# AugmentariumLab/VolumeRenderer

Hardware: AMD Instinct MI355X
Metric: Mvoxels/s kd-tree compress+decode (higher is better)
Workload: dtype u8; 1 GPU; 2048x2048x1920 uint8 volume per GPU as 960 bricks of 256x256x128, rm_volume, tolerance 1, maxEpochs 2, VolumeKdtree build + levelCut

## Files before the change

volumerenderer_amd/csrc/brickset.h:

```cpp
#pragma once
#include "kd_common.h"
#include "../../include/vrhip.h"
#include <algorithm>
#include <string>
#include <vector>

namespace vr {

struct Stream2 {
    uint8_t *temp = nullptr;
    uint8_t *codes = nullptr;
    uint8_t *recon[3] = {nullptr, nullptr, nullptr};
    Ctrl *ctrl = nullptr;
    uint8_t *tree = nullptr;
    uint8_t *treeCompact = nullptr;
};

struct Switches {
    bool decodeWalk = false;
    bool decodeFineV1 = false;
    bool decodeQuad = false;
    bool noSkipBlocks = false;
    bool noUniformBlocks = false;
    bool noUniformDecode = false;
};

#define VR_LOD_SLOTS 4
struct LodSlot {
    int32_t *dev = nullptr;
    int32_t *host = nullptr;
    uint8_t *idxValCut = nullptr;
    uint32_t *decTables = nullptr;
    uint8_t *rankVals = nullptr;
    int64_t *obDev = nullptr;
    int64_t *obHost = nullptr;
    vr_pool_entry *tabHost = nullptr;
    int64_t tabCap = 0;
    hipEvent_t done = nullptr;
    bool pending = false;
};

struct BrickSet {
    int32_t B = 0;
    Switches sw;
    Geom g{};
    TilePlan tile{};
// ... 108 lines not shown
```

volumerenderer_amd/csrc/capi.hip:

```cpp
#include "../../include/vrhip.h"
#include "brickset.h"
#include "raymarch.h"
#include <math.h>
#include <stdio.h>
#include <stdlib.h>
#include <string.h>
#include <algorithm>
#include <array>
#include <atomic>
#include <map>
#include <mutex>
#include <new>

using namespace vr;

struct vr_brickset { BrickSet s; };

#define HIPCHK(x) do { hipError_t e_ = (x); if (e_ != hipSuccess) return e_ == hipErrorOutOfMemory ? VR_ERR_OOM : VR_ERR_NO_DEVICE; } while (0)

static bool device_ok()
{
    int n = 0;
    hipError_t e = hipGetDeviceCount(&n);
    if ((e != hipSuccess || n <= 0) && getenv("VRHIP_DEBUG"))
// ... 186 lines not shown
static bool misaligned16(const void *p) { return ((uintptr_t)p & 15) != 0; }

vr_status vr_brickset_create(vr_brickset **out, int32_t num_bricks, const int64_t dims[3], int32_t tolerance,
                             int32_t max_epochs, int32_t variant)
{
    if (!out || !dims || num_bricks <= 0) return VR_ERR_INVALID;
    if (tolerance < 0 || max_epochs < 0 || variant < 0 || variant > 2) return VR_ERR_INVALID;
    for (int k = 0; k < 3; ++k) if (dims[k] <= 0) return VR_ERR_INVALID;
    bool general = !pow2(dims[0]) || !pow2(dims[1]) || !pow2(dims[2]) || dims[0] > 1024 || dims[1] > 1024 || dims[2] > 1024;
    if (dims[0] > (1ll << 20) || dims[1] > (1ll << 20) || dims[2] > (1ll << 20) || dims[0] * dims[1] * dims[2] >= (1ll << 32))
        return VR_ERR_UNSUPPORTED;
    if (!device_ok()) return VR_ERR_NO_DEVICE;
    vr_brickset *h = new (std::nothrow) vr_brickset();
    if (!h) return VR_ERR_OOM;
    BrickSet &b = h->s;
    b.B = num_bricks;
    {
        Switches &w = b.sw;
        w.decodeWalk = getenv("VRHIP_DECODE_WALK") != nullptr;
        w.decodeFineV1 = getenv("VRHIP_DECODE_FINE_V1") != nullptr;
        w.decodeQuad = getenv("VRHIP_DECODE_QUAD") != nullptr;
        w.noSkipBlocks = getenv("VRHIP_NO_SKIP_BLOCKS") != nullptr;
        w.noUniformBlocks = getenv("VRHIP_NO_UNIFORM_BLOCKS") != nullptr;
        w.noUniformDecode = getenv("VRHIP_NO_UNIFORM_DECODE") != nullptr;
    }
    make_geom(b.g, dims);
    b.D = b.g.D;
    if (b.D > 31) { delete h; return VR_ERR_UNSUPPORTED; }
    b.idx64 = b.D > 28 || (getenv("VRHIP_FORCE_IDX64") && b.D >= 12);
    if (b.idx64) general = true;
    if (b.idx64 && num_bricks != 1 && b.D > 28) { delete h; return VR_ERR_UNSUPPORTED; }
    b.generalGeom = general;
    b.maxDepth = b.D + VR_CHAIN_LEVELS;
    b.tolerance = tolerance; b.maxEpochs = max_epochs; b.variant = variant;
    b.K = b.D < 6 ? b.D : 6;
    b.Ds = b.D - b.K;
    b.heapStride = (int64_t)1 << (b.D + 1);
    b.leafStride = (int64_t)1 << b.D;
    b.codeStride = ((b.heapStride + 15) / 16) * 4;
    b.reconStride = b.leafStride;
    const int64_t numMax = b.heapStride - 1 + VR_CHAIN_LEVELS * b.leafStride;
    b.treeCap = ((numMax + 15) / 16 + 2) * 4 + 256;
    if (b.D >= 12) {
        const int64_t gappedBytes = ((int64_t)1 << (b.D - 12)) * 2320 * 4 + 256;
        if (gappedBytes > b.treeCap) b.treeCap = gappedBytes;
    }
// ... 15 lines not shown
        if (e == hipSuccess && !general) e = upload(b.lut, make_lut(b.g, b.K));
        if (e == hipSuccess && !general) e = hipMalloc(&b.spread, (size_t)(b.g.X + b.g.Y + b.g.Z) * sizeof(uint32_t));
        if (e == hipSuccess && !general) e = upload(b.spread, make_spread(b.g));
        for (int i = 0; i < 8 && e == hipSuccess; ++i) e = hipEventCreate(&b.ev[i]);
        if (e != hipSuccess) rc = e == hipErrorOutOfMemory ? VR_ERR_OOM : VR_ERR_NO_DEVICE;
    }
    if (rc != VR_OK) { vr_brickset_destroy(h); return rc; }
    b.hostCtrl.resize(b.B);
    b.openTreeBytes.assign(b.B, -1);
    *out = h;
    return VR_OK;
}

vr_status vr_brickset_set_switch(vr_brickset *h, const char *name, int32_t value)
{
    if (!h || !name) return VR_ERR_INVALID;
    Switches &w = h->s.sw;
    const bool on = value != 0;
    if (!strcmp(name, "decode_walk")) w.decodeWalk = on;
    else if (!strcmp(name, "decode_fine_v1")) w.decodeFineV1 = on;
    else if (!strcmp(name, "decode_quad")) w.decodeQuad = on;
    else if (!strcmp(name, "no_skip_blocks")) w.noSkipBlocks = on;
    else if (!strcmp(name, "no_uniform_blocks")) w.noUniformBlocks = on;
    else if (!strcmp(name, "no_uniform_decode")) w.noUniformDecode = on;
    else return VR_ERR_INVALID;
    return VR_OK;
}

vr_status vr_brickset_set_compaction(vr_brickset *h, int32_t on_build)
{
    if (!h) return VR_ERR_INVALID;
    h->s.compactOnBuild = on_build != 0;
    return VR_OK;
}

vr_status vr_debug_set(const char *name, int32_t value)
{
    if (!name) return VR_ERR_INVALID;
    if (!strcmp(name, "skip_grid_v1")) { vr::g_skipGridV1.store(value ? 1 : 0); return VR_OK; }
    if (!strcmp(name, "reslice_tile_w")) {
        if (value != 8 && value != 16 && value != 64) return VR_ERR_INVALID;
        vr::g_resliceTileLog2.store(value == 8 ? 3 : (value == 16 ? 4 : 6));
        return VR_OK;
    }
    if (!strcmp(name, "hist_plain")) { vr::g_histPlain.store(value ? 1 : 0); return VR_OK; }
    return VR_ERR_INVALID;
// ... 1019 lines not shown
```

volumerenderer_amd/csrc/kd_encode.hip:

```cpp
#include "brickset.h"
#include <math.h>
#include <stdio.h>
#include <stdlib.h>
#include <string.h>

namespace vr {

#define FILL_NODES_PER_BLOCK 1024
#define EMIT_RANKS_PER_BLOCK 256

template <bool FROM_VOXELS>
__global__ void __launch_bounds__(256)
k_pyramid(Geom g, int dLeaf, int L, const uint8_t *__restrict__ vox, const uint8_t *__restrict__ inMin,
          const uint8_t *__restrict__ inMax, int64_t inStride, uint8_t *__restrict__ temp, int64_t heapStride,
          uint8_t *__restrict__ tempRange, uint8_t *__restrict__ outMin, uint8_t *__restrict__ outMax,
          int64_t outStride, const uint32_t *__restrict__ srcIdx)
{
    __shared__ uint8_t smn[2][1024], smx[2][1024];
    const int brick = blockIdx.y;
    const uint32_t n = 1u << L;
    const uint32_t base = blockIdx.x << L;
    uint8_t *T = temp + (int64_t)brick * heapStride;
    uint8_t *TR = tempRange ? tempRange + (int64_t)brick * heapStride : nullptr;
    for (uint32_t i = threadIdx.x; i < n; i += blockDim.x) {
// ... 225 lines not shown
            const uint32_t u = pk_u(__builtin_elementwise_min(pk_s(waveMM[2 * h]), pk_s(waveMM[2 * h + 1])));
            a[h] = (int)(u & 0xFFFFu); b[h] = 255 - (int)(u >> 16);
            const int64_t o = ((int64_t)1 << (D - 11)) + (base >> 11) + h;
            T[o] = (uint8_t)((a[h] + b[h]) >> 1);
            if (TR) TR[o] = (uint8_t)((b[h] - a[h]) >> 1);
        }
        const int ra = min(a[0], a[1]), rbm = max(b[0], b[1]);
        const int64_t o = ((int64_t)1 << (D - 12)) + (base >> 12);
        T[o] = (uint8_t)((ra + rbm) >> 1);
        if (TR) TR[o] = (uint8_t)((rbm - ra) >> 1);
        outMin[(int64_t)brick * outStride + (base >> 12)] = (uint8_t)ra;
        outMax[(int64_t)brick * outStride + (base >> 12)] = (uint8_t)rbm;
        if (blockFlag) blockFlag[(int64_t)brick * ((int64_t)1 << (D - 12)) + (base >> 12)] = ra == rbm ? 1u : 0u;
        if (blockFlagR) blockFlagR[(int64_t)brick * ((int64_t)1 << (D - 12)) + (base >> 12)] = ra == rbm ? 1u : 0u;
    }
}

struct ReconBufs { uint8_t *b[3]; };

struct SkipBlocks {
    uint8_t *flag;
    int64_t nBlk;
    int Dm2;
};
__device__ __forceinline__ bool skip_block(const SkipBlocks &sk, int brick, int d, uint32_t node)
{
    return sk.flag && d > sk.Dm2 && (sk.flag[(int64_t)brick * sk.nBlk + (node >> (10 + d - sk.Dm2))] & 2u) != 0u;
}

__device__ inline int phys_buf(const Ctrl &c, int role) { return role == 0 ? c.ra : c.rb; }

__global__ void k_ctrl_init(Ctrl *ctrls, const uint8_t *rootMin, const uint8_t *rootMax, int64_t mmStride)
{
    Ctrl &c = ctrls[blockIdx.x];
    if (threadIdx.x) return;
    c.constBrick = 0; c.constVal = 0; c.zeroRun = 0;
    if (rootMin) {
        const int mn = rootMin[(int64_t)blockIdx.x * mmStride], mx = rootMax[(int64_t)blockIdx.x * mmStride];
        c.constBrick = mn == mx ? 1 : 0;
        c.constVal = mn;
    }
    c.currentDistance = c.currentError = c.currentDF = c.currentStepSize = 0.0;
    c.previousDistance = c.previousError = c.previousDF = c.previousStepSize = 0.0;
    c.errMinus = c.errPlus = 0;
    c.statL1 = 0;
    c.numActive = 0;
    c.epoch = 0; c.active = 0; c.fillThisEpoch = 0;
    c.cur = 0; c.prev = 1; c.pendingEqual = 0;
    c.par = 0; c.ra = 1; c.rb = 2;
    c.altValid = 0; c.altSel = 0; c.altDist = 0;
// ... 10 lines not shown
#define est_at(ci, seg) (((int64_t)(ci) * summStride + (int64_t)(seg)) * 4)

__device__ __forceinline__ uint32_t wave_incl_scan_u32(uint32_t v, int lane)
{
    (void)lane;
    return wave_incl_scan_add_dpp(v);
}

__device__ __forceinline__ uint32_t lane_u32(uint32_t v, int l) { return (uint32_t)__builtin_amdgcn_readlane((int)v, l); }
__device__ __forceinline__ unsigned long long lane_u64(unsigned long long v, int l)
{
    return (unsigned long long)lane_u32((uint32_t)v, l) | ((unsigned long long)lane_u32((uint32_t)(v >> 32), l) << 32);
}

#define EST_STAGE_NODES 4096
__device__ inline void est_exact_chain(const uint8_t *__restrict__ T, const uint8_t *__restrict__ P, int d, uint32_t lo,
                                       uint32_t hi, unsigned long long &S, uint32_t &C, int lane, const SkipBlocks &sk, int brick,
                                       uint8_t *stage = nullptr)
{
    const uint32_t len = hi - lo;
    const bool staged = stage && d > 0 && len >= 64u && len <= (uint32_t)EST_STAGE_NODES && (len & 63u) == 0u && (lo & 31u) == 0u;
    const uint8_t *sT = stage, *sP = stage + EST_STAGE_NODES;
    if (staged) {
        for (uint32_t i = (uint32_t)lane * 16u; i < len; i += 1024u) *(uint4 *)(stage + i) = *(const uint4 *)(T + lo + i);
        for (uint32_t i = (uint32_t)lane * 16u; i < len / 2u; i += 1024u) *(uint4 *)(stage + EST_STAGE_NODES + i) = *(const uint4 *)(P + (lo >> 1) + i);
    }
    const bool sk0 = skip_block(sk, brick, d, lo);
    int tn = 0, pn = 0;
    if (staged) { tn = sT[lane]; pn = sP[lane >> 1]; }
    else { tn = (!sk0 && lo + lane < hi) ? T[lo + lane] : 0; pn = (!sk0 && lo + lane < hi && d > 0) ? P[(lo + lane) >> 1] : 0; }
    bool skipThis = sk0;
    for (uint32_t base = lo; base < hi; base += 64) {
        uint32_t i = base + lane;
        bool valid = i < hi;
        const int t = tn, p = pn;
        const bool skipped = skipThis;
        {
            const uint32_t i2 = i + 64;
            skipThis = base + 64 < hi && skip_block(sk, brick, d, base + 64);
            if (staged) {
                const uint32_t j2 = i2 - lo;
                tn = j2 < len ? sT[j2] : 0;
                pn = j2 < len ? sP[j2 >> 1] : 0;
            } else {
                tn = (!skipThis && i2 < hi) ? T[i2] : 0;
                pn = (!skipThis && i2 < hi && d > 0) ? P[i2 >> 1] : 0;
            }
        }
        if (skipped) continue;
        int pd = p > t ? p - t : t - p;
        bool forced = (t > p && 2 * t - p > 255) || (t < p && 2 * t < p);
        bool cand = valid && pd > 0;
        bool dec = cand && (forced || S < (unsigned long long)pd * (2ull * C + 1ull));
        unsigned long long mask = __ballot(dec);
        for (int it = 0; it < 65; ++it) {
            uint32_t cpre = __popcll(mask & ((1ull << lane) - 1ull));
            uint32_t v = dec ? (uint32_t)pd : 0u;
            uint32_t spre = wave_incl_scan_u32(v, lane) - v;
            bool nd = cand && (forced || (S + spre) < (unsigned long long)pd * (2ull * (C + cpre) + 1ull));
            unsigned long long nmask = __ballot(nd);
            dec = nd;
            if (nmask == mask) break;
            mask = nmask;
        }
        S += (uint32_t)__builtin_amdgcn_readlane((int)wave_incl_scan_add_dpp(dec ? (uint32_t)pd : 0u), 63);
        C += __popcll(mask);
    }
}

// ... 49 lines not shown
    return v + dpp_u32<0x142, 0xa>(0, v);
}
__device__ __forceinline__ int seg_max_i32_dpp(int v)
{
    v = row_max_i32_dpp(v);
    return max(v, (int)dpp_u32<0x142, 0xa>(0x80000000u, (uint32_t)v));
}
__device__ __forceinline__ int seg_min_i32_dpp(int v)
{
    v = row_min_i32_dpp(v);
    return min(v, (int)dpp_u32<0x142, 0xa>(0x7FFFFFFFu, (uint32_t)v));
}

__global__ void __launch_bounds__(256)
k_est_summ(int d, int nc, Ctrl *ctrls, const uint8_t *__restrict__ temp, int64_t heapStride, ReconBufs rb,
           int64_t leafStride, uint32_t *__restrict__ summ, int64_t summStride, SkipBlocks sk)
{
    constexpr int L = 32, SPW = 64 / L, NP = EST_SEG / 2 / L, TW = NP / 2, PW = NP / 4;
    const int brick = blockIdx.y, lane = threadIdx.x & 63, row = lane / L, rl = lane % L;
    const Ctrl &c = ctrls[brick];
    const uint32_t n = 1u << d;
    const int cConst = c.constBrick, cDone = c.estDone, cSeg = c.estSeg, cPar = c.par, cTbase = c.estTbase;
    if (cConst || cDone) return;
    const uint8_t *Tl = temp + (int64_t)brick * heapStride + ((int64_t)1 << d) + rl * (4 * TW);
    const uint8_t *Pl = (cPar == 0 ? rb.b[0] : (cPar == 1 ? rb.b[1] : rb.b[2])) + (int64_t)brick * leafStride + rl * (4 * PW);
    const uint32_t nseg = n / EST_SEG, step = gridDim.x * (4u * SPW);
    const uint32_t g0 = (uint32_t)cSeg + (blockIdx.x * 4u + (threadIdx.x >> 6)) * SPW;
    uint4 tN[TW / 4], pN[PW / 4];
    auto fetch = [&](uint32_t g) {
        const uint32_t s = g + (uint32_t)row;
        const bool live = s < nseg && !skip_block(sk, brick, d, s * EST_SEG);
#pragma unroll
        for (int j = 0; j < TW / 4; ++j) tN[j] = make_uint4(0, 0, 0, 0);
#pragma unroll
        for (int j = 0; j < PW / 4; ++j) pN[j] = make_uint4(0, 0, 0, 0);
        if (live) {
#pragma unroll
            for (int j = 0; j < TW / 4; ++j) tN[j] = ld16(Tl + (size_t)s * EST_SEG + 16 * j);
#pragma unroll
            for (int j = 0; j < PW / 4; ++j) pN[j] = ld16(Pl + (size_t)s * (EST_SEG / 2) + 16 * j);
        }
    };
    fetch(g0);
    const int Tbase = cTbase;
    uint32_t *out = summ + (int64_t)brick * summStride * (4 * EST_CAND);
    for (uint32_t g = g0; g < nseg; g += step) {
    uint32_t tw[TW], pw[PW];
#pragma unroll
    for (int j = 0; j < TW / 4; ++j) { tw[4 * j] = tN[j].x; tw[4 * j + 1] = tN[j].y; tw[4 * j + 2] = tN[j].z; tw[4 * j + 3] = tN[j].w; }
#pragma unroll
    for (int j = 0; j < PW / 4; ++j) { pw[4 * j] = pN[j].x; pw[4 * j + 1] = pN[j].y; pw[4 * j + 2] = pN[j].z; pw[4 * j + 3] = pN[j].w; }
    const uint32_t seg = g + (uint32_t)row;
    const bool segLive = seg < nseg;
    uint32_t mixed = 0;
    {
        const uint32_t t0 = __builtin_amdgcn_perm(0, tw[0], 0u), p0 = __builtin_amdgcn_perm(0, pw[0], 0u);
#pragma unroll
        for (int j = 0; j < TW; ++j) mixed |= tw[j] ^ t0;
#pragma unroll
// ... 255 lines not shown
{
    __shared__ unsigned long long shm[4], shp[4];
    const int brick = blockIdx.y;
    Ctrl &c = ctrls[brick];
    const int cConst = c.constBrick, cFill = c.fillThisEpoch, cPar = c.par, cCur = c.cur, cRa = c.ra, cRb = c.rb, cEpoch = c.epoch;
    const double cDist = c.currentDistance;
    if (cConst || !cFill) return;
    if (!STORE && c.altSel) return;
    const uint8_t *T = temp + (int64_t)brick * heapStride + ((int64_t)1 << d);
    uint8_t *Cd = codes + (int64_t)brick * codeStride + ((int64_t)1 << (d - 2));
    const int rPhys = cCur == 0 ? cRa : cRb;
    const uint8_t *P = (cPar == 0 ? rb.b[0] : (cPar == 1 ? rb.b[1] : rb.b[2])) + (int64_t)brick * leafStride;
    uint8_t *R = (rPhys == 0 ? rb.b[0] : (rPhys == 1 ? rb.b[1] : rb.b[2])) + (int64_t)brick * leafStride;
    const int dist = (int)(uint8_t)cDist;
    const int distM = (int)(uint8_t)fmax(0.0, cDist - 1.0);
    const int distP = (int)(uint8_t)fmin(255.0, cDist + 1.0);
    const bool needDF = cEpoch + 1 < maxEpochs;
    const uint32_t d2 = (uint32_t)dist * 0x10001u, dm2 = (uint32_t)distM * 0x10001u, dp2 = (uint32_t)distP * 0x10001u;
    const int w = threadIdx.x >> 6;
    const uint32_t nchunk = (uint32_t)(((size_t)1 << d) >> 12);
    uint32_t chunk = blockIdx.x * (uint32_t)iters;
    const uint32_t chunkEnd = chunk + (uint32_t)iters < nchunk ? chunk + (uint32_t)iters : nchunk;
    unsigned long long accM = 0, accP = 0;
    bool skippedN = skip_block(sk, brick, d, (chunk * 4u + (uint32_t)w) << 10);
    uint4 tvN = make_uint4(0, 0, 0, 0);
    uint2 pvN = make_uint2(0, 0);
    if (!skippedN) { const size_t i0 = ((size_t)chunk * 256u + threadIdx.x) * 16u; tvN = ld16(T + i0); pvN = ld8(P + (i0 >> 1)); }
    for (; chunk < chunkEnd; ++chunk) {
    const size_t i0 = ((size_t)chunk * 256u + threadIdx.x) * 16u;
    const bool skipped = skippedN;
    const uint4 tv = tvN;
    const uint2 pv = pvN;
    if (chunk + 1 < chunkEnd) {
        skippedN = skip_block(sk, brick, d, ((chunk + 1u) * 4u + (uint32_t)w) << 10);
        tvN = make_uint4(0, 0, 0, 0); pvN = make_uint2(0, 0);
        if (!skippedN) { const size_t i1 = i0 + 4096u; tvN = ld16(T + i1); pvN = ld8(P + (i1 >> 1)); }
    }
    const uint32_t tw[4] = {tv.x, tv.y, tv.z, tv.w}, pw[2] = {pv.x, pv.y};
    uint32_t e0 = 0, em = 0, ep = 0, wa = 0, wb = 0, rw[4] = {tw[0], tw[1], tw[2], tw[3]}, rprev = 0;
    const uint32_t differs = (tw[0] ^ __builtin_amdgcn_perm(0, pw[0], 0x01010000u)) | (tw[1] ^ __builtin_amdgcn_perm(0, pw[0], 0x03030202u)) |
                             (tw[2] ^ __builtin_amdgcn_perm(0, pw[1], 0x01010000u)) | (tw[3] ^ __builtin_amdgcn_perm(0, pw[1], 0x03030202u));
    const bool busy = !skipped && __ballot(differs != 0u) != 0ull;
    if (sk.flag && d == sk.Dm2 && !busy && (threadIdx.x & 63) == 0) {
        uint8_t *f = sk.flag + (int64_t)brick * sk.nBlk + (size_t)chunk * 4 + w;
        if (*f & 1u) *f = 3u;
    }
    const auto pair = [&](const int j) {
        const EncPair c = enc_pair(tw[j >> 1], j & 1, pw[j >> 2], j & 3);
        const vr_s16x2 x = enc_pair_x(c, d2), ax = pk_abs(x);
        e0 = pk_sumsq(__builtin_elementwise_min(c.pd, ax), e0);
        if (STORE) {
        const uint32_t take = pk_u((ax - c.pd) >> 15);
        const uint32_t code2 = take & pk_u(pk_s(c.up) + pk_s(0x00020002u));
        if (j < 4) wa |= code2 << (4 * j); else wb |= code2 << (4 * (j - 4));
        const vr_s16x2 r = pk_mad(x, pk_mad(pk_s(c.up), pk_s(0xFFFEFFFEu), pk_s(0xFFFFFFFFu)), c.T2);
        const uint32_t rec = (take & pk_u(r)) | (~take & pk_u(c.P2));
        if (j & 1) rw[j >> 1] = __builtin_amdgcn_perm(rec, rprev, 0x06040200u); else rprev = rec;
        }
        if (needDF) {
            em = pk_sumsq(enc_pair_err(c, dm2), em);
            ep = pk_sumsq(enc_pair_err(c, dp2), ep);
        }
    };
    bool uniform = false;
    if (busy) {
        const uint32_t t0 = __builtin_amdgcn_perm(0, tw[0], 0u), p0 = __builtin_amdgcn_perm(0, pw[0], 0u);
        const uint32_t mixed = (tw[0] ^ t0) | (tw[1] ^ t0) | (tw[2] ^ t0) | (tw[3] ^ t0) | (pw[0] ^ p0) | (pw[1] ^ p0);
        uniform = __ballot(mixed != 0u) == 0ull;
    }
    if (uniform) {
        pair(0);
        e0 *= 8u; em *= 8u; ep *= 8u;
        if (STORE) {
            wa *= 0x1111u; wb = wa;
            rw[0] = rw[1] = rw[2] = rw[3] = __builtin_amdgcn_perm(0, rprev, 0u);
        }
    } else if (busy)
#pragma unroll
        for (int j = 0; j < 8; ++j) pair(j);
    const uint32_t cpk = ((wa | (wa >> 14)) & 0xFFFFu) | ((wb | (wb >> 14)) << 16);
    if (!skipped && STORE) {
        st4(Cd + (i0 >> 2), cpk);
        st16(R + i0, make_uint4(rw[0], rw[1], rw[2], rw[3]));
    }
    unsigned long long s0 = 0, sm = 0, sp = 0;
    if (busy) {
        s0 = (uint32_t)__builtin_amdgcn_readlane((int)wave_incl_scan_add_dpp(e0), 63);
        sm = (uint32_t)__builtin_amdgcn_readlane((int)wave_incl_scan_add_dpp(em), 63);
        sp = (uint32_t)__builtin_amdgcn_readlane((int)wave_incl_scan_add_dpp(ep), 63);
    }
    if ((threadIdx.x & 63) == 0) {
        blockErr[(int64_t)brick * nErrBlk + (size_t)chunk * 4 + w] = s0;
        if (!STORE && needDF) {
            blockErr[errPlane + (int64_t)brick * nErrBlk + (size_t)chunk * 4 + w] = sm;
            blockErr[2 * errPlane + (int64_t)brick * nErrBlk + (size_t)chunk * 4 + w] = sp;
        }
    }
    accM += sm; accP += sp;
    }
    if ((threadIdx.x & 63) == 0) { shm[w] = accM; shp[w] = accP; }
    __syncthreads();
    if (threadIdx.x == 0) {
        const unsigned long long tm = shm[0] + shm[1] + shm[2] + shm[3], tp = shp[0] + shp[1] + shp[2] + shp[3];
        if (tm) atomicAdd(&c.errMinus, tm);
// ... 25 lines not shown
            int er = encode_node(t, p, dist).err;
            e = (uint32_t)(er * er);
        }
        const uint32_t incl = wave_incl_scan_u32(e, lane);
        const uint32_t total = lane_u32(incl, 63);
        uint32_t consumed = 0;
        int start = 0;
        while (true) {
            bool ok = true;
            if (lane >= start && s != 0.0) ok = (s + (double)(incl - consumed)) < next_pow2_above(s);
            const unsigned long long bad = ~__ballot(ok);
            if (bad == 0ull) { s = s + (double)(total - consumed); break; }
            const int f = __ffsll((long long)bad) - 1;
            const uint32_t exclF = lane_u32(incl - e, f), eF = lane_u32(e, f);
            s = s + (double)(exclF - consumed);
            s = s + (double)eF;
            consumed = exclF + eF;
            start = f + 1;
        }
    }
    return s;
}

__device__ inline double ctl_walk_block16(double s, const uint8_t *__restrict__ T, const uint8_t *__restrict__ P, int dist,
                                          uint32_t lo, int lane)
{
    const uint4 tv = *(const uint4 *)(T + lo + lane * 16);
    const uint2 pv = *(const uint2 *)(P + (lo >> 1) + lane * 8);
    const uint32_t tw[4] = {tv.x, tv.y, tv.z, tv.w}, pw[2] = {pv.x, pv.y};
    const uint32_t d2 = (uint32_t)dist * 0x10001u;
    uint32_t e[16], pre[16];
    uint32_t run = 0;
#pragma unroll
    for (int j = 0; j < 8; ++j) {
        const EncPair c = enc_pair(tw[j >> 1], j & 1, pw[j >> 2], j & 3);
        const vr_s16x2 er = enc_pair_err(c, d2);
        e[2 * j] = (uint32_t)((int)er.x * (int)er.x);
        e[2 * j + 1] = (uint32_t)((int)er.y * (int)er.y);
        run += e[2 * j]; pre[2 * j] = run;
        run += e[2 * j + 1]; pre[2 * j + 1] = run;
    }
    const uint32_t inclL = wave_incl_scan_add_dpp(run);
    const uint32_t baseL = inclL - run, total = (uint32_t)__builtin_amdgcn_readlane((int)inclL, 63);
    uint32_t consumed = 0;
    int startPos = 0;
    while (true) {
        int fail = 16;
        if (s != 0.0) {
            const double bound = next_pow2_above(s);
#pragma unroll
            for (int k = 15; k >= 0; --k)
                if (lane * 16 + k >= startPos && !((s + (double)(baseL + pre[k] - consumed)) < bound)) fail = k;
        }
        const unsigned long long bad = __ballot(fail < 16);
        if (bad == 0ull) { s = s + (double)(total - consumed); break; }
        const int f = __ffsll((long long)bad) - 1;
        const int kF = __builtin_amdgcn_readlane(fail, f);
        uint32_t eF = 0, gF = 0;
#pragma unroll
        for (int k = 0; k < 16; ++k) if (k == kF) { eF = e[k]; gF = baseL + pre[k]; }
        eF = (uint32_t)__builtin_amdgcn_readlane((int)eF, f);
        gF = (uint32_t)__builtin_amdgcn_readlane((int)gF, f);
        s = s + (double)(gF - eF - consumed);
        s = s + (double)eF;
        consumed = gF;
        startPos = f * 16 + kF + 1;
    }
    return s;
}

#define CTL_STAGE_BLOCKS 8192
__device__ inline double ctl_partials64(double s, const unsigned long long *__restrict__ be, const uint32_t *stg, uint32_t base, uint32_t nblk,
                                        const uint8_t *__restrict__ T, const uint8_t *__restrict__ P, int d, int dist,
                                        uint32_t n, int lane)
{
    const unsigned long long e2 = base + lane < nblk ? (stg ? (unsigned long long)stg[base + lane] : be[base + lane]) : 0ull;
    const unsigned long long incl = (unsigned long long)wave_incl_scan_add_dpp((uint32_t)(e2 & 0xFFFFFFull)) +
                                    ((unsigned long long)wave_incl_scan_add_dpp((uint32_t)(e2 >> 24)) << 24);
    const unsigned long long total = lane_u64(incl, 63);
    unsigned long long consumed = 0;
    int start = 0;
    while (true) {
        bool ok = true;
        const bool sInt = (s == floor(s)) && (s + (double)(total - consumed)) < 9007199254740992.0;
        if (lane >= start && !sInt) ok = (s + (double)(incl - consumed)) < next_pow2_above(s);
        const unsigned long long bad = ~__ballot(ok);
        if (bad == 0ull) { s = s + (double)(total - consumed); break; }
        const int f = __ffsll((long long)bad) - 1;
        const unsigned long long exclF = lane_u64(incl - e2, f), inclF = lane_u64(incl, f);
        s = s + (double)(exclF - consumed);
        uint32_t lo = (base + f) * FILL_NODES_PER_BLOCK, hi = lo + FILL_NODES_PER_BLOCK;
        if (hi > n) hi = n;
        s = (hi - lo == 1024u && d > 0) ? ctl_walk_block16(s, T, P, dist, lo, lane) : ctl_walk_block(s, T, P, d, dist, lo, hi, lane);
        consumed = inclF;
        start = f + 1;
    }
    return s;
}

__global__ void __launch_bounds__(64)
k_control(int d, int maxEpochs, int guarded, Ctrl *ctrls, const uint8_t *__restrict__ temp, int64_t heapStride,
          ReconBufs rb, int64_t leafStride, const unsigned long long *__restrict__ blockErr, int64_t nErrBlk, int64_t errPlane,
          int leaflessLeaf)
{
    const int brick = blockIdx.x, lane = threadIdx.x;
    __shared__ __attribute__((aligned(16))) uint32_t ctlStage[CTL_STAGE_BLOCKS];
    Ctrl &c = ctrls[brick];
    if (c.constBrick) return;
    const uint32_t n = 1u << d;
    const bool ending = c.active && c.fillThisEpoch;
    double s = c.currentError;
    if (ending) {
        const uint8_t *T = temp + (int64_t)brick * heapStride + ((int64_t)1 << d);
        const uint8_t *P = rb.b[c.par] + (int64_t)brick * leafStride;
        const int dist = (int)(uint8_t)c.currentDistance;
        const uint32_t nblk = (n + FILL_NODES_PER_BLOCK - 1) / FILL_NODES_PER_BLOCK;
        const unsigned long long *be = blockErr + (int64_t)c.altSel * errPlane + (int64_t)brick * nErrBlk;
        const uint32_t nchunk = (nblk + 63u) >> 6;
        const uint32_t *stg = nullptr;
        if (nblk >= 256u && nblk <= (uint32_t)CTL_STAGE_BLOCKS && (nblk & 255u) == 0u) {
            for (uint32_t i = (uint32_t)lane * 4u; i < nblk; i += 256u) {
                const uint4 a = *(const uint4 *)(be + i), b = *(const uint4 *)(be + i + 2);
                *(uint4 *)(ctlStage + i) = make_uint4(a.x, a.z, b.x, b.z);
            }
            stg = ctlStage;
        }
// ... 7 lines not shown
            } else if (ch < nchunk) {
                const unsigned long long *q = be + (size_t)ch * 64;
                const uint32_t m = nblk - ch * 64 < 64u ? nblk - ch * 64 : 64u;
                if (m == 64u) {
#pragma unroll 8
                    for (int k = 0; k < 64; ++k) tot += q[k];
                } else
                    for (uint32_t k = 0; k < m; ++k) tot += q[k];
            }
            const unsigned long long incl = (unsigned long long)wave_incl_scan_add_dpp((uint32_t)(tot & 0xFFFFFFull)) +
                                            ((unsigned long long)wave_incl_scan_add_dpp((uint32_t)(tot >> 24)) << 24);
            const unsigned long long total = lane_u64(incl, 63);
            unsigned long long consumed = 0;
            int start = 0;
            while (true) {
                bool ok = true;
                const bool sInt = (s == floor(s)) && (s + (double)(total - consumed)) < 9007199254740992.0;
                if (lane >= start && !sInt) ok = (s + (double)(incl - consumed)) < next_pow2_above(s);
                const unsigned long long bad = ~__ballot(ok);
                if (bad == 0ull) { s = s + (double)(total - consumed); break; }
                const int f = __ffsll((long long)bad) - 1;
                const unsigned long long exclF = lane_u64(incl - tot, f), inclF = lane_u64(incl, f);
                s = s + (double)(exclF - consumed);
                s = ctl_partials64(s, be, stg, (cb + (uint32_t)f) * 64u, nblk, T, P, d, dist, n, lane);
                consumed = inclF;
                start = f + 1;
            }
        }
    }
    if (lane != 0) return;
    if (ending) {
        c.roleDist[c.cur] = (int)(uint8_t)c.currentDistance;
        c.codesDist = (int)(uint8_t)c.currentDistance;
        c.altValid = leaflessLeaf && !c.altSel && c.epoch + 1 < maxEpochs;
        c.altDist = (int)(uint8_t)c.currentDistance;
        c.altSel = 0;
        c.currentError = s / (double)n;
        if (c.currentError < 1.0) {
            c.active = 0;
        } else if (c.epoch != 0 && c.currentError > c.previousError) {
            c.currentError = c.previousError;
            c.currentDistance = c.previousDistance;
            c.currentDF = c.previousDF;
            c.currentStepSize = c.previousStepSize / 2.0;
            int tmp = c.cur; c.cur = c.prev; c.prev = tmp;
            c.pendingEqual = 0;
            c.numReverts++;
// ... 1390 lines not shown

static void compress_stream(BrickSet *bs, Stream2 &s0, hipStream_t st, const uint8_t *rootMin, const uint8_t *rootMax,
                            int64_t mmStride, SkipBlocks sk, unsigned long long *blockErr, void *estSumm0,
                            int b0 = 0, int nb = -1)
{
    const int D = bs->D, B = nb < 0 ? bs->B : nb;
    struct { Ctrl *ctrl; uint8_t *temp, *codes; uint8_t *recon[3]; } s;
    s.ctrl = s0.ctrl + b0; s.temp = s0.temp + (int64_t)b0 * bs->heapStride; s.codes = s0.codes + (int64_t)b0 * bs->codeStride;
    for (int i = 0; i < 3; ++i) s.recon[i] = s0.recon[i] + (int64_t)b0 * bs->reconStride;
    blockErr += (int64_t)b0 * bs->nErrBlk;
    const int64_t errPlane = (int64_t)bs->B * bs->nErrBlk;
    void *estSumm = (uint32_t *)estSumm0 + (int64_t)b0 * bs->estSummStride * (4 * EST_CAND);
    if (sk.flag) sk.flag += (int64_t)b0 * sk.nBlk;
    if (rootMin) { rootMin += (int64_t)b0 * mmStride; rootMax += (int64_t)b0 * mmStride; }
    ReconBufs rb{{s.recon[0], s.recon[1], s.recon[2]}};
    const int guarded = bs->variant != 0;
    hipLaunchKernelGGL(k_ctrl_init, dim3(B), dim3(64), 0, st, s.ctrl, rootMin, rootMax, mmStride);
    if (bs->maxEpochs <= 0) {
        for (int i = 0; i < 3; ++i) hipMemsetAsync(s.recon[i], 0, (size_t)B * bs->reconStride, st);
        hipMemsetAsync(s.codes, 0, (size_t)B * bs->codeStride, st);
    }
    for (int d = 0; d <= D; ++d) {
        const int64_t n = (int64_t)1 << d;
        if (sk.flag && d == D - 1)
            hipLaunchKernelGGL(k_fill_const_leaves, dim3(cdiv(sk.nBlk, 256), B), dim3(256), 0, st, D, s.ctrl, s.temp,
                               bs->heapStride, sk);
        hipLaunchKernelGGL(k_est_head, dim3(B), dim3(64), 0, st, d, bs->maxEpochs, s.ctrl, s.temp, bs->heapStride, rb,
                           bs->reconStride, sk);
        if (n > EST_HEAD) {
            const int64_t nseg = n / EST_SEG - EST_HEAD / EST_SEG;
            for (int r = 0; r < EST_ROUNDS; ++r) {
                const int nc = r < 2 ? 4 : EST_CAND, ncNext = r + 1 < 2 ? 4 : EST_CAND;
                const unsigned gx = r == 0 ? cdiv(nseg, 32) : (cdiv(nseg, 8) < 64 ? cdiv(nseg, 8) : 64);
                hipLaunchKernelGGL(k_est_summ, dim3(gx, B), dim3(256), 0, st, d, nc, s.ctrl, s.temp,
                                   bs->heapStride, rb, bs->reconStride, (uint32_t *)estSumm, bs->estSummStride, sk);
                hipLaunchKernelGGL(k_est_walk, dim3(B), dim3(64), 0, st, d, bs->maxEpochs, nc, ncNext,
                                   r == EST_ROUNDS - 1 ? 1 : 0, s.ctrl, s.temp, bs->heapStride, rb, bs->reconStride,
                                   (const uint32_t *)estSumm, bs->estSummStride, sk);
            }
        }
        for (int e = 0; e < bs->maxEpochs; ++e) {
            if (n >= 4096)
            {
                const int iters = n / 4096 >= 512 ? FILL_ITERS : (n / 4096 >= 64 ? (FILL_ITERS < 4 ? FILL_ITERS : 4) : 1);
                hipLaunchKernelGGL((bs->leafless && d == D) ? k_fill16<false> : k_fill16<true>, dim3(cdiv(n / 4096, iters), B), dim3(256), 0, st,
                                   d, bs->maxEpochs, s.ctrl, s.temp, s.codes, bs->heapStride, bs->codeStride, rb, bs->reconStride, blockErr,
                                   bs->nErrBlk, sk, errPlane, iters);
            }
            else
                hipLaunchKernelGGL(k_fill, dim3(cdiv(n, FILL_NODES_PER_BLOCK), B), dim3(256), 0, st, d, s.ctrl, s.temp,
                                   s.codes, bs->heapStride, bs->codeStride, rb, bs->reconStride, blockErr, bs->nErrBlk);
            hipLaunchKernelGGL(k_control, dim3(B), dim3(64), 0, st, d, bs->maxEpochs, guarded, s.ctrl, s.temp,
                               bs->heapStride, rb, bs->reconStride, blockErr, bs->nErrBlk, errPlane, (bs->leafless && d == D) ? 1 : 0);
        }
        hipLaunchKernelGGL(k_level_end, dim3(B), dim3(64), 0, st, d, s.ctrl);
    }
}

__global__ void k_fix_chain_distances(int D, int maxDepth, Ctrl *ctrls, Ctrl *ctrlsR)
{
    if (threadIdx.x) return;
    const int add[VR_CHAIN_LEVELS] = {64, 32, 16, 8, 4, 2, 1};
    for (int dd = D + 1, i = 0; dd <= maxDepth; ++dd, ++i) {
        ctrls[blockIdx.x].distanceMap[dd] = (uint8_t)add[i];
        if (ctrlsR) ctrlsR[blockIdx.x].distanceMap[dd] = (uint8_t)add[i];
    }
}

static bool dbg_sync(hipStream_t st, const char *phase)
{
    static const bool on = getenv("VRHIP_SYNC") != nullptr;
    if (!on) return true;
    hipError_t e = hipStreamSynchronize(st);
    fprintf(stderr, "[vrhip] phase %s: %s\n", phase, hipGetErrorString(e));
    return e == hipSuccess;
}
// ... 96 lines not shown
        while (dLeaf > 0 || round == 0) {
            int L = dLeaf < 10 ? dLeaf : 10;
            int64_t nblk = (int64_t)1 << (dLeaf - L);
            uint8_t *oMin = bs->mmMin[round & 1], *oMax = bs->mmMax[round & 1];
            if (round == 0)
                hipLaunchKernelGGL(k_pyramid<true>, dim3((unsigned)nblk, B), dim3(256), 0, st, bs->g, dLeaf, L, vox,
                                   inMin, inMax, inStride, bs->mid.temp, bs->heapStride, mr ? bs->rng.temp : nullptr,
                                   oMin, oMax, oStride, bs->generalGeom ? bs->srcIdx : nullptr);
            else
                hipLaunchKernelGGL(k_pyramid<false>, dim3((unsigned)nblk, B), dim3(256), 0, st, bs->g, dLeaf, L, vox,
                                   inMin, inMax, inStride, bs->mid.temp, bs->heapStride, mr ? bs->rng.temp : nullptr,
                                   oMin, oMax, oStride, nullptr);
            dLeaf -= L;
            rootMinP = oMin; rootMaxP = oMax;
            if (dLeaf == 0) break;
            inMin = oMin; inMax = oMax; inStride = oStride;
            ++round;
        }
    }
    hipEventRecord(bs->ev[1], st);
    dbg_sync(st, "pyramid");
    const bool constOk = bs->maxEpochs >= 1 && bs->tolerance >= 1 && D >= 1;
    const uint8_t *cMin = constOk ? rootMinP : nullptr, *cMax = constOk ? rootMaxP : nullptr;
    const SkipBlocks sk{skipOn ? bs->blockFlag : nullptr, (int64_t)1 << (D >= 12 ? D - 12 : 0), D - 2};
    const SkipBlocks skR{skipOn && mr ? bs->blockFlagR : nullptr, sk.nBlk, D - 2};
    const bool forkR = mr && bs->blockErrR && bs->estSummR && ensure_aux(bs, 1) == 1;
    if (forkR) {
        hipEventRecord(bs->evFork, st);
        hipStreamWaitEvent(bs->aux, bs->evFork, 0);
        compress_stream(bs, bs->rng, bs->aux, cMin, cMax, rootStride, skR, bs->blockErrR, bs->estSummR);
        hipEventRecord(bs->evJoin, bs->aux);
    }
    int parts = bs->levelLoopStreams;
    if (parts > 4) parts = 4;
    if (mr || B < 16 * parts || parts < 2) parts = 1;
    if (parts > 1) parts = 1 + ensure_aux(bs, parts - 1);
    if (parts > 1) {
        hipEventRecord(bs->evFork, st);
        for (int p = 1; p < parts; ++p) {
            const int b0 = (int)((int64_t)B * p / parts), b1 = (int)((int64_t)B * (p + 1) / parts);
            hipStreamWaitEvent(bs->auxN[p - 1], bs->evFork, 0);
            compress_stream(bs, bs->mid, bs->auxN[p - 1], cMin, cMax, rootStride, sk, bs->blockErr, bs->estSumm, b0, b1 - b0);
            hipEventRecord(bs->evJoinN[p - 1], bs->auxN[p - 1]);
        }
        compress_stream(bs, bs->mid, st, cMin, cMax, rootStride, sk, bs->blockErr, bs->estSumm, 0, (int)((int64_t)B / parts));
        for (int p = 1; p < parts; ++p) hipStreamWaitEvent(st, bs->evJoinN[p - 1], 0);
    } else
    compress_stream(bs, bs->mid, st, cMin, cMax, rootStride, sk, bs->blockErr, bs->estSumm);
// ... 5 lines not shown
    ReconBufs rb{{bs->mid.recon[0], bs->mid.recon[1], bs->mid.recon[2]}};
    ReconBufs rbR{{bs->rng.recon[0], bs->rng.recon[1], bs->rng.recon[2]}};
    int pruneFrom = D - 1;
    bs->fineHas.assign((size_t)B, 0);
    fine_has_changed(*bs);
    if (fused) {
        PruneEmitArgs pa;
        pa.sk = sk; pa.skR = skR;
        pa.D = D; pa.tol = bs->tolerance; pa.maxDepth = bs->maxDepth; pa.ctrls = bs->mid.ctrl;
        pa.temp = bs->mid.temp; pa.codes = bs->mid.codes;
        pa.heapStride = bs->heapStride; pa.codeStride = bs->codeStride; pa.leafStride = bs->reconStride;
        pa.rb = rb; pa.subTok = bs->blockOff; pa.nEmitBlk = bs->nEmitBlk; pa.blockL1 = bs->blockL1;
        pa.chainLut = bs->chainLut; pa.idxOff = bs->idxOff; pa.nIdx = bs->nIdx;
        if (!bs->fineIdx && hipMalloc(&bs->fineIdx, (size_t)B * bs->nIdx * 16) != hipSuccess) return -3;
        if (!bs->idxVal3 && hipMalloc(&bs->idxVal3, (size_t)B * bs->nIdx * 8) != hipSuccess) return -3;
        const size_t boxBytes = (size_t)B * ((size_t)1 << (D - 12)) * sizeof(uint32_t);
        if (!bs->boxUniform && hipMalloc(&bs->boxUniform, boxBytes) != hipSuccess) return -3;
        if (hipMemsetAsync(bs->boxUniform, 0, boxBytes, st) != hipSuccess) return -1;
        pa.fineIdx = (uint32_t *)bs->fineIdx; pa.boxUniform = bs->boxUniform;
        pa.ctrlsR = mr ? bs->rng.ctrl : nullptr; pa.tempR = mr ? bs->rng.temp : nullptr; pa.codesR = mr ? bs->rng.codes : nullptr;
        pa.rbR = rbR;
        pa.gap = bs->mid.tree; pa.gapR = mr ? bs->rng.tree : nullptr; pa.treeCap = bs->treeCap;
        const dim3 peGrid((unsigned)((int64_t)1 << (D - 12)), B);
        pa.uniformBlocks = skipOn && bs->leafless && !mr && !bs->sw.noUniformBlocks;
        if (pa.uniformBlocks)
            hipLaunchKernelGGL(k_prune_emit12_const, dim3((unsigned)cdiv((int64_t)1 << (D - 12), PEC_BOXES), B), dim3(256), 0, st, pa);
        if (bs->leafless) {
            hipLaunchKernelGGL((k_prune_emit12<false, true>), peGrid, dim3(256), 0, st, pa);
            if (mr) hipLaunchKernelGGL((k_prune_emit12<true, true>), peGrid, dim3(256), 0, st, pa);
        } else {
            hipLaunchKernelGGL((k_prune_emit12<false, false>), peGrid, dim3(256), 0, st, pa);
            if (mr) hipLaunchKernelGGL((k_prune_emit12<true, false>), peGrid, dim3(256), 0, st, pa);
        }
        pruneFrom = D - 13;
        bs->fineHas.assign((size_t)B, 1);
        fine_has_changed(*bs);
    } else
        hipLaunchKernelGGL(k_prune_leaf, dim3(cdiv((int64_t)1 << D, 256), B), dim3(256), 0, st, D, bs->tolerance,
                           bs->mid.ctrl, bs->mid.temp, bs->mid.codes, mr ? bs->rng.codes : nullptr, bs->heapStride,
                           bs->codeStride, rb, bs->reconStride, bs->maxDepth, bs->blockL1, bs->nEmitBlk);
    for (int d = pruneFrom; d >= 0; --d)
        hipLaunchKernelGGL(k_prune_level, dim3(cdiv((int64_t)1 << d, 256), B), dim3(256), 0, st, d, bs->mid.ctrl, bs->mid.codes,
                           mr ? bs->rng.codes : nullptr, bs->codeStride);
    hipLaunchKernelGGL(k_fix_chain_distances, dim3(B), dim3(64), 0, st, D, bs->maxDepth, bs->mid.ctrl,
                       mr ? bs->rng.ctrl : nullptr);
    hipEventRecord(bs->ev[3], st);
    dbg_sync(st, "prune");
// ... 30 lines not shown
```

Before: 280,700 Mvoxels/s.

## Synthesize constant-box values in level loop instead of loading heap data

Adds a levelConst mode to SkipBlocks. Boxes flagged uniform (flag bit 1) are treated as constant at the D-2 level and below: the estimate, fill and control kernels read a single scalar per box and broadcast it instead of loading T/P rows, and stores are limited to the first chunk of each constant box. The separate k_fill_const_leaves pass is skipped when this mode is on. It aims to cut memory traffic on uniform regions. In exchange it adds per-access flag lookups and branches, and correctness depends on constant boxes really being uniform across all levels.

```diff
diff --git a/volumerenderer_amd/csrc/brickset.h b/volumerenderer_amd/csrc/brickset.h
--- a/volumerenderer_amd/csrc/brickset.h
+++ b/volumerenderer_amd/csrc/brickset.h
@@ -22,6 +22,7 @@
     bool decodeQuad = false;
     bool noSkipBlocks = false;
     bool noUniformBlocks = false;
+    bool noLevelConstBoxes = false;
     bool noUniformDecode = false;
 };
 
diff --git a/volumerenderer_amd/csrc/capi.hip b/volumerenderer_amd/csrc/capi.hip
--- a/volumerenderer_amd/csrc/capi.hip
+++ b/volumerenderer_amd/csrc/capi.hip
@@ -232,6 +232,7 @@
         w.decodeQuad = getenv("VRHIP_DECODE_QUAD") != nullptr;
         w.noSkipBlocks = getenv("VRHIP_NO_SKIP_BLOCKS") != nullptr;
         w.noUniformBlocks = getenv("VRHIP_NO_UNIFORM_BLOCKS") != nullptr;
+        w.noLevelConstBoxes = getenv("VRHIP_NO_LEVEL_CONST_BOXES") != nullptr;
         w.noUniformDecode = getenv("VRHIP_NO_UNIFORM_DECODE") != nullptr;
     }
     make_geom(b.g, dims);
@@ -293,6 +294,7 @@
     else if (!strcmp(name, "decode_quad")) w.decodeQuad = on;
     else if (!strcmp(name, "no_skip_blocks")) w.noSkipBlocks = on;
     else if (!strcmp(name, "no_uniform_blocks")) w.noUniformBlocks = on;
+    else if (!strcmp(name, "no_level_const_boxes")) w.noLevelConstBoxes = on;
     else if (!strcmp(name, "no_uniform_decode")) w.noUniformDecode = on;
     else return VR_ERR_INVALID;
     return VR_OK;
diff --git a/volumerenderer_amd/csrc/kd_encode.hip b/volumerenderer_amd/csrc/kd_encode.hip
--- a/volumerenderer_amd/csrc/kd_encode.hip
+++ b/volumerenderer_amd/csrc/kd_encode.hip
@@ -271,10 +271,33 @@
     uint8_t *flag;
     int64_t nBlk;
     int Dm2;
+    int levelConst;
 };
 __device__ __forceinline__ bool skip_block(const SkipBlocks &sk, int brick, int d, uint32_t node)
 {
     return sk.flag && d > sk.Dm2 && (sk.flag[(int64_t)brick * sk.nBlk + (node >> (10 + d - sk.Dm2))] & 2u) != 0u;
+}
+__device__ __forceinline__ int box_kind(const SkipBlocks &sk, int brick, int d, uint32_t node, uint32_t &box)
+{
+    if (!sk.flag || d < sk.Dm2 || (d == sk.Dm2 && !sk.levelConst)) return 0;
+    box = node >> (10 + d - sk.Dm2);
+    const uint32_t f = sk.flag[(int64_t)brick * sk.nBlk + box];
+    if (d > sk.Dm2 && (f & 2u) != 0u) return 1;
+    return (sk.levelConst && (f & 1u) != 0u) ? 2 : 0;
+}
+__device__ __forceinline__ void box_scalars(const SkipBlocks &sk, const uint8_t *__restrict__ T, const uint8_t *__restrict__ P, int d,
+                                            uint32_t box, uint32_t &v, uint32_t &p)
+{
+    v = T[((int64_t)1 << (sk.Dm2 - 10)) - ((int64_t)1 << d) + (int64_t)box];
+    p = P[(size_t)box << (9 + d - sk.Dm2)];
+}
+__device__ __forceinline__ bool box_scalars_at(const SkipBlocks &sk, int brick, const uint8_t *__restrict__ T, const uint8_t *__restrict__ P,
+                                               int d, uint32_t node, uint32_t &v, uint32_t &p)
+{
+    uint32_t box = 0;
+    if (box_kind(sk, brick, d, node, box) != 2) return false;
+    box_scalars(sk, T, P, d, box, v, p);
+    return true;
 }
 
 __device__ inline int phys_buf(const Ctrl &c, int role) { return role == 0 ? c.ra : c.rb; }
@@ -331,13 +354,30 @@
     const bool staged = stage && d > 0 && len >= 64u && len <= (uint32_t)EST_STAGE_NODES && (len & 63u) == 0u && (lo & 31u) == 0u;
     const uint8_t *sT = stage, *sP = stage + EST_STAGE_NODES;
     if (staged) {
-        for (uint32_t i = (uint32_t)lane * 16u; i < len; i += 1024u) *(uint4 *)(stage + i) = *(const uint4 *)(T + lo + i);
-        for (uint32_t i = (uint32_t)lane * 16u; i < len / 2u; i += 1024u) *(uint4 *)(stage + EST_STAGE_NODES + i) = *(const uint4 *)(P + (lo >> 1) + i);
-    }
+        uint32_t v = 0, p = 0;
+        for (uint32_t i = (uint32_t)lane * 16u; i < len; i += 1024u) {
+            const bool cb = box_scalars_at(sk, brick, T, P, d, lo + i, v, p);
+            const uint32_t v4 = v * 0x01010101u;
+            *(uint4 *)(stage + i) = cb ? make_uint4(v4, v4, v4, v4) : *(const uint4 *)(T + lo + i);
+        }
+        for (uint32_t i = (uint32_t)lane * 16u; i < len / 2u; i += 1024u) {
+            const bool cb = box_scalars_at(sk, brick, T, P, d, lo + 2u * i, v, p);
+            const uint32_t p4 = p * 0x01010101u;
+            *(uint4 *)(stage + EST_STAGE_NODES + i) = cb ? make_uint4(p4, p4, p4, p4) : *(const uint4 *)(P + (lo >> 1) + i);
+        }
+    }
+    const auto direct = [&](uint32_t i, bool skippedChunk, int &t, int &p) {
+        t = 0; p = 0;
+        if (skippedChunk || i >= hi) return;
+        uint32_t v = 0, q = 0;
+        if (box_scalars_at(sk, brick, T, P, d, i, v, q)) { t = (int)v; p = (int)q; return; }
+        t = T[i];
+        if (d > 0) p = P[i >> 1];
+    };
     const bool sk0 = skip_block(sk, brick, d, lo);
     int tn = 0, pn = 0;
     if (staged) { tn = sT[lane]; pn = sP[lane >> 1]; }
-    else { tn = (!sk0 && lo + lane < hi) ? T[lo + lane] : 0; pn = (!sk0 && lo + lane < hi && d > 0) ? P[(lo + lane) >> 1] : 0; }
+    else direct(lo + lane, sk0, tn, pn);
     bool skipThis = sk0;
     for (uint32_t base = lo; base < hi; base += 64) {
         uint32_t i = base + lane;
@@ -352,8 +392,7 @@
                 tn = j2 < len ? sT[j2] : 0;
                 pn = j2 < len ? sP[j2 >> 1] : 0;
             } else {
-                tn = (!skipThis && i2 < hi) ? T[i2] : 0;
-                pn = (!skipThis && i2 < hi && d > 0) ? P[i2 >> 1] : 0;
+                direct(i2, skipThis, tn, pn);
             }
         }
         if (skipped) continue;
@@ -449,19 +488,28 @@
     const uint32_t n = 1u << d;
     const int cConst = c.constBrick, cDone = c.estDone, cSeg = c.estSeg, cPar = c.par, cTbase = c.estTbase;
     if (cConst || cDone) return;
-    const uint8_t *Tl = temp + (int64_t)brick * heapStride + ((int64_t)1 << d) + rl * (4 * TW);
-    const uint8_t *Pl = (cPar == 0 ? rb.b[0] : (cPar == 1 ? rb.b[1] : rb.b[2])) + (int64_t)brick * leafStride + rl * (4 * PW);
+    const uint8_t *T = temp + (int64_t)brick * heapStride + ((int64_t)1 << d), *Tl = T + rl * (4 * TW);
+    const uint8_t *P = (cPar == 0 ? rb.b[0] : (cPar == 1 ? rb.b[1] : rb.b[2])) + (int64_t)brick * leafStride, *Pl = P + rl * (4 * PW);
     const uint32_t nseg = n / EST_SEG, step = gridDim.x * (4u * SPW);
     const uint32_t g0 = (uint32_t)cSeg + (blockIdx.x * 4u + (threadIdx.x >> 6)) * SPW;
     uint4 tN[TW / 4], pN[PW / 4];
     auto fetch = [&](uint32_t g) {
         const uint32_t s = g + (uint32_t)row;
-        const bool live = s < nseg && !skip_block(sk, brick, d, s * EST_SEG);
+        uint32_t box = 0;
+        const int kind = s < nseg ? box_kind(sk, brick, d, s * EST_SEG, box) : 1;
 #pragma unroll
         for (int j = 0; j < TW / 4; ++j) tN[j] = make_uint4(0, 0, 0, 0);
 #pragma unroll
         for (int j = 0; j < PW / 4; ++j) pN[j] = make_uint4(0, 0, 0, 0);
-        if (live) {
+        if (kind == 2) {
+            uint32_t v, p;
+            box_scalars(sk, T, P, d, box, v, p);
+            v *= 0x01010101u; p *= 0x01010101u;
+#pragma unroll
+            for (int j = 0; j < TW / 4; ++j) tN[j] = make_uint4(v, v, v, v);
+#pragma unroll
+            for (int j = 0; j < PW / 4; ++j) pN[j] = make_uint4(p, p, p, p);
+        } else if (kind == 0) {
 #pragma unroll
             for (int j = 0; j < TW / 4; ++j) tN[j] = ld16(Tl + (size_t)s * EST_SEG + 16 * j);
 #pragma unroll
@@ -763,20 +811,27 @@
     uint32_t chunk = blockIdx.x * (uint32_t)iters;
     const uint32_t chunkEnd = chunk + (uint32_t)iters < nchunk ? chunk + (uint32_t)iters : nchunk;
     unsigned long long accM = 0, accP = 0;
-    bool skippedN = skip_block(sk, brick, d, (chunk * 4u + (uint32_t)w) << 10);
-    uint4 tvN = make_uint4(0, 0, 0, 0);
-    uint2 pvN = make_uint2(0, 0);
-    if (!skippedN) { const size_t i0 = ((size_t)chunk * 256u + threadIdx.x) * 16u; tvN = ld16(T + i0); pvN = ld8(P + (i0 >> 1)); }
+    int kindN = 0;
+    uint4 tvN;
+    uint2 pvN;
+    const auto fetch = [&](uint32_t ch) {
+        uint32_t box = 0;
+        kindN = box_kind(sk, brick, d, (ch * 4u + (uint32_t)w) << 10, box);
+        tvN = make_uint4(0, 0, 0, 0); pvN = make_uint2(0, 0);
+        if (kindN == 2) {
+            uint32_t v, p;
+            box_scalars(sk, T, P, d, box, v, p);
+            v *= 0x01010101u; p *= 0x01010101u;
+            tvN = make_uint4(v, v, v, v); pvN = make_uint2(p, p);
+        } else if (kindN == 0) { const size_t i1 = ((size_t)ch * 256u + threadIdx.x) * 16u; tvN = ld16(T + i1); pvN = ld8(P + (i1 >> 1)); }
+    };
+    fetch(chunk);
     for (; chunk < chunkEnd; ++chunk) {
     const size_t i0 = ((size_t)chunk * 256u + threadIdx.x) * 16u;
-    const bool skipped = skippedN;
+    const bool skipped = kindN == 1, constBox = kindN == 2;
     const uint4 tv = tvN;
     const uint2 pv = pvN;
-    if (chunk + 1 < chunkEnd) {
-        skippedN = skip_block(sk, brick, d, ((chunk + 1u) * 4u + (uint32_t)w) << 10);
-        tvN = make_uint4(0, 0, 0, 0); pvN = make_uint2(0, 0);
-        if (!skippedN) { const size_t i1 = i0 + 4096u; tvN = ld16(T + i1); pvN = ld8(P + (i1 >> 1)); }
-    }
+    if (chunk + 1 < chunkEnd) fetch(chunk + 1u);
     const uint32_t tw[4] = {tv.x, tv.y, tv.z, tv.w}, pw[2] = {pv.x, pv.y};
     uint32_t e0 = 0, em = 0, ep = 0, wa = 0, wb = 0, rw[4] = {tw[0], tw[1], tw[2], tw[3]}, rprev = 0;
     const uint32_t differs = (tw[0] ^ __builtin_amdgcn_perm(0, pw[0], 0x01010000u)) | (tw[1] ^ __builtin_amdgcn_perm(0, pw[0], 0x03030202u)) |
@@ -820,7 +875,7 @@
 #pragma unroll
         for (int j = 0; j < 8; ++j) pair(j);
     const uint32_t cpk = ((wa | (wa >> 14)) & 0xFFFFu) | ((wb | (wb >> 14)) << 16);
-    if (!skipped && STORE) {
+    if (!skipped && STORE && (!constBox || (i0 & (((size_t)1024 << (d - sk.Dm2)) - 1u)) == 0u)) {
         st4(Cd + (i0 >> 2), cpk);
         st16(R + i0, make_uint4(rw[0], rw[1], rw[2], rw[3]));
     }
@@ -892,11 +947,19 @@
     return s;
 }
 
-__device__ inline double ctl_walk_block16(double s, const uint8_t *__restrict__ T, const uint8_t *__restrict__ P, int dist,
-                                          uint32_t lo, int lane)
-{
-    const uint4 tv = *(const uint4 *)(T + lo + lane * 16);
-    const uint2 pv = *(const uint2 *)(P + (lo >> 1) + lane * 8);
+__device__ inline double ctl_walk_block16(double s, const uint8_t *__restrict__ T, const uint8_t *__restrict__ P, int d, int dist,
+                                          uint32_t lo, int lane, const SkipBlocks &sk, int brick)
+{
+    uint4 tv;
+    uint2 pv;
+    uint32_t v = 0, p = 0;
+    if (box_scalars_at(sk, brick, T, P, d, lo, v, p)) {
+        v *= 0x01010101u; p *= 0x01010101u;
+        tv = make_uint4(v, v, v, v); pv = make_uint2(p, p);
+    } else {
+        tv = *(const uint4 *)(T + lo + lane * 16);
+        pv = *(const uint2 *)(P + (lo >> 1) + lane * 8);
+    }
     const uint32_t tw[4] = {tv.x, tv.y, tv.z, tv.w}, pw[2] = {pv.x, pv.y};
     const uint32_t d2 = (uint32_t)dist * 0x10001u;
     uint32_t e[16], pre[16];
@@ -942,7 +1005,7 @@
 #define CTL_STAGE_BLOCKS 8192
 __device__ inline double ctl_partials64(double s, const unsigned long long *__restrict__ be, const uint32_t *stg, uint32_t base, uint32_t nblk,
                                         const uint8_t *__restrict__ T, const uint8_t *__restrict__ P, int d, int dist,
-                                        uint32_t n, int lane)
+                                        uint32_t n, int lane, const SkipBlocks &sk, int brick)
 {
     const unsigned long long e2 = base + lane < nblk ? (stg ? (unsigned long long)stg[base + lane] : be[base + lane]) : 0ull;
     const unsigned long long incl = (unsigned long long)wave_incl_scan_add_dpp((uint32_t)(e2 & 0xFFFFFFull)) +
@@ -961,7 +1024,7 @@
         s = s + (double)(exclF - consumed);
         uint32_t lo = (base + f) * FILL_NODES_PER_BLOCK, hi = lo + FILL_NODES_PER_BLOCK;
         if (hi > n) hi = n;
-        s = (hi - lo == 1024u && d > 0) ? ctl_walk_block16(s, T, P, dist, lo, lane) : ctl_walk_block(s, T, P, d, dist, lo, hi, lane);
+        s = (hi - lo == 1024u && d > 0) ? ctl_walk_block16(s, T, P, d, dist, lo, lane, sk, brick) : ctl_walk_block(s, T, P, d, dist, lo, hi, lane);
         consumed = inclF;
         start = f + 1;
     }
@@ -971,7 +1034,7 @@
 __global__ void __launch_bounds__(64)
 k_control(int d, int maxEpochs, int guarded, Ctrl *ctrls, const uint8_t *__restrict__ temp, int64_t heapStride,
           ReconBufs rb, int64_t leafStride, const unsigned long long *__restrict__ blockErr, int64_t nErrBlk, int64_t errPlane,
-          int leaflessLeaf)
+          int leaflessLeaf, SkipBlocks sk)
 {
     const int brick = blockIdx.x, lane = threadIdx.x;
     __shared__ __attribute__((aligned(16))) uint32_t ctlStage[CTL_STAGE_BLOCKS];
@@ -1025,7 +1088,7 @@
                 const int f = __ffsll((long long)bad) - 1;
                 const unsigned long long exclF = lane_u64(incl - tot, f), inclF = lane_u64(incl, f);
                 s = s + (double)(exclF - consumed);
-                s = ctl_partials64(s, be, stg, (cb + (uint32_t)f) * 64u, nblk, T, P, d, dist, n, lane);
+                s = ctl_partials64(s, be, stg, (cb + (uint32_t)f) * 64u, nblk, T, P, d, dist, n, lane, sk, brick);
                 consumed = inclF;
                 start = f + 1;
             }
@@ -2462,7 +2525,7 @@
     }
     for (int d = 0; d <= D; ++d) {
         const int64_t n = (int64_t)1 << d;
-        if (sk.flag && d == D - 1)
+        if (sk.flag && !sk.levelConst && d == D - 1)
             hipLaunchKernelGGL(k_fill_const_leaves, dim3(cdiv(sk.nBlk, 256), B), dim3(256), 0, st, D, s.ctrl, s.temp,
                                bs->heapStride, sk);
         hipLaunchKernelGGL(k_est_head, dim3(B), dim3(64), 0, st, d, bs->maxEpochs, s.ctrl, s.temp, bs->heapStride, rb,
@@ -2491,7 +2554,7 @@
                 hipLaunchKernelGGL(k_fill, dim3(cdiv(n, FILL_NODES_PER_BLOCK), B), dim3(256), 0, st, d, s.ctrl, s.temp,
                                    s.codes, bs->heapStride, bs->codeStride, rb, bs->reconStride, blockErr, bs->nErrBlk);
             hipLaunchKernelGGL(k_control, dim3(B), dim3(64), 0, st, d, bs->maxEpochs, guarded, s.ctrl, s.temp,
-                               bs->heapStride, rb, bs->reconStride, blockErr, bs->nErrBlk, errPlane, (bs->leafless && d == D) ? 1 : 0);
+                               bs->heapStride, rb, bs->reconStride, blockErr, bs->nErrBlk, errPlane, (bs->leafless && d == D) ? 1 : 0, sk);
         }
         hipLaunchKernelGGL(k_level_end, dim3(B), dim3(64), 0, st, d, s.ctrl);
     }
@@ -2634,8 +2697,10 @@
     dbg_sync(st, "pyramid");
     const bool constOk = bs->maxEpochs >= 1 && bs->tolerance >= 1 && D >= 1;
     const uint8_t *cMin = constOk ? rootMinP : nullptr, *cMax = constOk ? rootMaxP : nullptr;
-    const SkipBlocks sk{skipOn ? bs->blockFlag : nullptr, (int64_t)1 << (D >= 12 ? D - 12 : 0), D - 2};
-    const SkipBlocks skR{skipOn && mr ? bs->blockFlagR : nullptr, sk.nBlk, D - 2};
+    const bool uniformBlocks = skipOn && bs->leafless && !mr && !bs->sw.noUniformBlocks;
+    const SkipBlocks sk{skipOn ? bs->blockFlag : nullptr, (int64_t)1 << (D >= 12 ? D - 12 : 0), D - 2,
+                        uniformBlocks && !bs->sw.noLevelConstBoxes ? 1 : 0};
+    const SkipBlocks skR{skipOn && mr ? bs->blockFlagR : nullptr, sk.nBlk, D - 2, 0};
     const bool forkR = mr && bs->blockErrR && bs->estSummR && ensure_aux(bs, 1) == 1;
     if (forkR) {
         hipEventRecord(bs->evFork, st);
@@ -2687,7 +2752,7 @@
         pa.rbR = rbR;
         pa.gap = bs->mid.tree; pa.gapR = mr ? bs->rng.tree : nullptr; pa.treeCap = bs->treeCap;
         const dim3 peGrid((unsigned)((int64_t)1 << (D - 12)), B);
-        pa.uniformBlocks = skipOn && bs->leafless && !mr && !bs->sw.noUniformBlocks;
+        pa.uniformBlocks = uniformBlocks;
         if (pa.uniformBlocks)
             hipLaunchKernelGGL(k_prune_emit12_const, dim3((unsigned)cdiv((int64_t)1 << (D - 12), PEC_BOXES), B), dim3(256), 0, st, pa);
         if (bs->leafless) {
```

Measured after the change: 281,400 Mvoxels/s, median of 6. Within noise of the previous version (+0.2%).
